# iqbal-lab-org/gramtools

Measured on AMD Instinct MI355X. Metric: 150bp reads quasimapped/sec (whole node); bit-exact coverage, higher is better.
Workload: dtype u32

## Files before the change

### gramtools_amd/csrc/gmx_engine_cover_kernels.h

```cpp
#pragma once
struct CoverAcc {
  uint32_t *acc;
  uint32_t *log;
  uint32_t *log_cursor;
  uint32_t log_cap;
  uint32_t *scratch_big;
  uint32_t n_lanes_big;
  int rng_mode;
  uint32_t log_sites;
  uint32_t *heap;
  uint64_t heap_words;
  const uint32_t *status;
  uint32_t n_tasks;
  unsigned long long *stats;
};

#define GMX_LOG_PAD 0xFFFFFFFFu
#ifdef GMX_LOOP_STATS
__device__ unsigned long long gmx_cover_stats[6 * 16];
__device__ unsigned long long gmx_coop_stats[6 * 8];
extern "C" int gmx_debug_coop_stats(unsigned long long *out, int reset) {
  if (hipMemcpyFromSymbol(out, HIP_SYMBOL(gmx_coop_stats), sizeof(gmx_coop_stats)) != hipSuccess) return -1;
  if (reset) {
    unsigned long long z[6 * 8] = {0};
// ... 808 lines not shown
    gmx_cover_single_rec<NESTED>(ix, o, acc, recs_in[i], o.cover_overflow_list, 4u);
}

__global__ void gmx_stats_limbs_kernel(unsigned long long *stats, uint32_t *limbs, int recombine) {
  const uint32_t t = threadIdx.x;
  if (!recombine) {
    if (t < 20) limbs[t] = (uint32_t)((stats[t >> 2] >> (16 * (t & 3))) & 0xFFFFull);
    else if (t < 32) limbs[t] = 0;
  } else if (t < 5) {
    unsigned long long v = 0;
    for (int l = 3; l >= 0; --l) v = (v << 16) + limbs[4 * t + l];
    stats[t] = v;
  }
}

#define GMX_PACK_READS 128
#define GMX_PACK_IN_BYTES (24 * 1024)
#define GMX_PACK_OUT_PAIRS (GMX_PACK_IN_BYTES / 32 + GMX_PACK_READS + 8)
typedef uint32_t __attribute__((aligned(1))) gmx_u32_unaligned;
__device__ __forceinline__ void pack4(uint32_t x, uint32_t &lo, uint32_t &hi, uint32_t &bad) {
  uint32_t y = x - 0x01010101u;
  bad |= ((y & ~x & 0x80808080u) | (y & 0xFCFCFCFCu));
  lo = (((y & 0x01010101u) * 0x01020408u) >> 24) & 0xFu;
  hi = ((((y >> 1) & 0x01010101u) * 0x01020408u) >> 24) & 0xFu;
}
__device__ __forceinline__ uint2 pack_tail(const uint8_t *p, uint32_t rem, uint32_t &bad) {
  uint2 out = make_uint2(0, 0);
  for (uint32_t j = 0; j < rem; ++j) {
    uint32_t x = p[j];
    if (x < 1 || x > 4) bad = 1;
    out.x |= ((x - 1u) & 1u) << j;
    out.y |= (((x - 1u) >> 1) & 1u) << j;
  }
  return out;
}
#define GMX_PACK_THREADS (2 * GMX_PACK_READS)
__global__ void __launch_bounds__(GMX_PACK_THREADS) gmx_pack_kernel(BatchView b, uint8_t *skip, uint2 *packed, uint32_t *counters,
                                                                    uint32_t *zero, uint32_t zero_words) {
  __shared__ uint4 in4[GMX_PACK_IN_BYTES / 16 + 2];
  __shared__ uint2 outp[GMX_PACK_OUT_PAIRS];
  if (blockIdx.x == 0)
    for (uint32_t i = threadIdx.x; i < GMX_N_COUNTERS * GMX_CNT_STRIDE; i += GMX_PACK_THREADS) counters[i] = 0;
  for (uint32_t i = blockIdx.x * GMX_PACK_THREADS + threadIdx.x; i < zero_words; i += gridDim.x * GMX_PACK_THREADS) zero[i] = 0;
  const uint32_t r0 = blockIdx.x * GMX_PACK_READS;
  const uint32_t r1 = min(r0 + GMX_PACK_READS, b.n_reads);
  const uint32_t read = r0 + (threadIdx.x >> 1), half = threadIdx.x & 1u;
  const uint64_t s0 = b.offsets[r0], s1 = b.offsets[r1];
  const uintptr_t g0 = reinterpret_cast<uintptr_t>(b.reads + s0);
  const uint32_t shift = (uint32_t)(g0 & 15u);
  const uint64_t span = (s1 - s0) + shift;
  if (span <= GMX_PACK_IN_BYTES) {
    const uint4 *src = reinterpret_cast<const uint4 *>(g0 - shift);
    const uint32_t n16 = (uint32_t)((span + 15) >> 4);
    {
      uint32_t i = threadIdx.x;
      for (; i + 2 * GMX_PACK_THREADS < n16; i += 3 * GMX_PACK_THREADS) {
        const uint4 v0 = src[i], v1 = src[i + GMX_PACK_THREADS], v2 = src[i + 2 * GMX_PACK_THREADS];
        in4[i] = v0;
// ... 66 lines not shown
```

### gramtools_amd/csrc/gmx_engine_debug.h

```cpp

struct GmxDebugPools {
  GmxFinalState *states = nullptr;
  uint32_t *stack = nullptr;
  GmxPathNode *arena = nullptr;
  uint32_t *result = nullptr;
  uint32_t *in = nullptr;
  uint2 *planes = nullptr;
  uint32_t cap_states = 0, cap_nodes = 0, cap_in = 0, cap_pairs = 0;
};

__global__ void __launch_bounds__(64) gmx_debug_search_kernel(GmxIndexView ix, BatchView b, const uint32_t *in, uint32_t from, uint32_t stop,
                                                              uint32_t mode, uint32_t from_seed_table, BigOut g, uint32_t *result) {
  const bool active = threadIdx.x == 0;
  BigCtx ctx;
  ctx.sp = 0;
  ctx.cap = g.max_states;
  ctx.stack = g.stack;
  ctx.arena = g.arena;
  ctx.arena_n = 0;
  ctx.arena_cap = g.max_path_nodes;
  ctx.status = GMX_TASK_MAPPED;
  ctx.out = g.states;
  ctx.n_out = 0;
  ctx.out_cap = g.max_states;
// ... 160 lines not shown
  }
  e->keep_states = on != 0;
  return GMX_OK;
} GMX_GUARD_INT("gmx_engine_debug_keep_states")

int gmx_debug_final_states(gmx_engine *e, uint64_t task, uint32_t *out, uint64_t cap_words, uint64_t *n_words, int *tier) try {
  if (!e || !n_words) {
    gmx_set_error("gmx_debug_final_states: null argument");
    return GMX_EINVAL;
  }
  if (!e->keep_states || task >= 2 * e->keep_reads) {
    gmx_set_error("gmx_debug_final_states: no such task in the last batch (gmx_engine_debug_keep_states first)");
    return GMX_EINVAL;
  }
  HIP_TRY(hipSetDevice(e->opts.device));
  HIP_TRY(hipDeviceSynchronize());
  int rc = debug_isa(e);
  if (rc) return rc;
  uint32_t raw[GMX_N_COUNTERS * GMX_CNT_STRIDE];
  HIP_TRY(hipMemcpy(raw, e->d_counters, sizeof(raw), hipMemcpyDeviceToHost));
  auto c = [&](int i) { return raw[i * GMX_CNT_STRIDE]; };
  DebugWriter w{out, cap_words};
  {
    const uint32_t n_huge = c(11);
    std::vector<uint32_t> huge(n_huge);
    if (n_huge) HIP_TRY(hipMemcpy(huge.data(), e->d_huge, n_huge * sizeof(uint32_t), hipMemcpyDeviceToHost));
    for (uint32_t t : huge)
      if (t == task) {
        gmx_set_error("gmx_debug_final_states: the task was searched by the last tier, which keeps no states");
        return GMX_ECAP;
// ... 247 lines not shown
```

### gramtools_amd/csrc/gmx_engine_host.h

```cpp
#pragma once
#define HIP_TRY(expr)                                                                      \
  do {                                                                                     \
    hipError_t _e = (expr);                                                                \
    if (_e != hipSuccess) {                                                                \
      gmx_set_error(std::string(#expr) + ": " + hipGetErrorString(_e));                    \
      return GMX_EHIP;                                                                     \
    }                                                                                      \
  } while (0)

enum : int { GMX_TK_SEED = 0, GMX_TK_FILTER0, GMX_TK_FILTER1, GMX_TK_SINGLE, GMX_TK_EXTEND2, GMX_TK_UNPACK, GMX_TK_N };
static_assert(GMX_TK_N <= GMX_TIMED_KERNELS, "gmx_timing::kernel_ms holds GMX_TIMED_KERNELS entries");

struct gmx_engine {
  gmx_engine_opts opts;
  GmxIndexView dview;
  std::vector<void *> allocs;
  uint64_t index_bytes = 0;
  uint32_t *d_fused = nullptr, *d_limbs = nullptr;
  size_t n_fused = 0, n_acc = 0;
  std::vector<uint32_t> phys_allele, phys_pb, phys_grouped;
  std::vector<uint32_t> hit_fix;
  unsigned long long *d_stats = nullptr;
  uint32_t *d_error = nullptr;
  uint32_t *d_log = nullptr, *d_log_cursor = nullptr;
// ... 33 lines not shown
  std::map<std::vector<uint32_t>, uint64_t> log_counts;
  uint32_t *h_log_state = nullptr;
  hipEvent_t ev_log_state = nullptr;
  bool log_state_pending = false;
  uint32_t *d_log_retry[2] = {nullptr, nullptr}, *d_log_retry_recs[2] = {nullptr, nullptr}, *d_log_retry_huge[2] = {nullptr, nullptr};
  int log_retry_side = 0;
  BatchView last_b{};
  SearchOut last_o{};
  CoverAcc last_acc{};
  size_t last_big_lds = 0;
  uint64_t log_replays = 0, log_replayed_entries = 0;
  uint64_t log_known = 0;
  uint64_t log_reads_since = 0;
  bool reset_pending = false;
  hipStream_t reset_stream = nullptr;
  hipStream_t side2_stream = nullptr;
  hipEvent_t ev_fork2 = nullptr, ev_side1 = nullptr, ev_filter = nullptr;
  hipStream_t side_stream = nullptr;
  hipEvent_t ev_fork = nullptr, ev_join = nullptr;
  hipEvent_t ev_wait = nullptr;
  struct GmxDeviceIndex *shared_index = nullptr;
  uint32_t filter_lds_words = 0;
  const uint32_t *d_kmer_planar = nullptr;
  const uint32_t *d_absent = nullptr;
  uint32_t n_absent = 0;
  bool use_absent = false;
  uint32_t n_cus = 256;
  uint32_t probe_iters = GMX_PROBE_ITERS;
  uint32_t extend_cap = 0;
  uint32_t extend_budget = 8;
// ... 85 lines not shown
    return GMX_OK;
  }
  int upload(const uint32_t **dst, const gmx::WordBuf &src) {
    uint32_t *q = nullptr;
    int rc = alloc(&q, src.size(), false);
    if (rc) return rc;
    const size_t piece = (size_t)1 << 28;
    for (size_t at = 0; at < src.size(); at += piece)
      HIP_TRY(hipMemcpy(q + at, src.data() + at, std::min(piece, src.size() - at) * sizeof(uint32_t), hipMemcpyHostToDevice));
    index_bytes += src.size() * sizeof(uint32_t);
    *dst = q;
    return GMX_OK;
  }
};

static hipError_t gmx_event_wait(hipEvent_t ev) {
  static const bool spin = getenv("GMX_WAIT_SPIN") != nullptr;
  if (spin) return hipEventSynchronize(ev);
  const auto t0 = std::chrono::steady_clock::now();
  for (bool napping = false;;) {
    const hipError_t q = hipEventQuery(ev);
    if (q != hipErrorNotReady) return q;
    (void)hipGetLastError();
    if (!napping) {
      napping = std::chrono::steady_clock::now() - t0 > std::chrono::microseconds(60);
      continue;
    }
    struct timespec ts = {0, 50 * 1000};
    nanosleep(&ts, nullptr);
  }
}

static int gmx_quiesce(gmx_engine *e) {
  if (!e->ev_wait) HIP_TRY(hipEventCreateWithFlags(&e->ev_wait, hipEventDisableTiming | hipEventBlockingSync));
  hipStream_t streams[5] = {e->last_stream, e->copy_stream, e->side_stream, e->side2_stream, e->copy_stream2};
  for (int i = 0; i < 5; ++i) {
    if (i > 0 && !streams[i]) continue;
    bool seen = false;
    for (int j = 0; j < i; ++j) seen = seen || streams[j] == streams[i];
    if (seen) continue;
// ... 9 lines not shown
  HIP_TRY(hipEventRecord(e->ev_zeroed, stream));
  ++e->zero_epoch;
  return GMX_OK;
}
static int twin_join(gmx_engine *e, hipStream_t stream) {
  gmx_engine *tw = e->twin;
  if (!tw || !e->twin_in_flight) return GMX_OK;
  if (!e->ev_twin_done) HIP_TRY(hipEventCreateWithFlags(&e->ev_twin_done, hipEventDisableTiming));
  HIP_TRY(hipEventRecord(e->ev_twin_done, tw->main_stream));
  HIP_TRY(hipStreamWaitEvent(stream, e->ev_twin_done, 0));
  return GMX_OK;
}
static int flush_reset(gmx_engine *e) {
  if (!e->reset_pending) return GMX_OK;
  e->reset_pending = false;
  HIP_TRY(hipMemsetAsync(e->d_fused, 0, (e->n_fused + 32) * 4, e->reset_stream));
  return note_zeroed(e, e->reset_stream);
}

static int log_settle(gmx_engine *e);
static int gmx_log_drain(gmx_engine *e, uint64_t keep_below) {
  int frc = flush_reset(e);
  if (frc) return frc;
  HIP_TRY(hipDeviceSynchronize());
  uint32_t used = 0;
  HIP_TRY(hipMemcpy(&used, e->d_log_cursor, 4, hipMemcpyDeviceToHost));
  used = std::min(used, e->log_cap);
  e->log_reads_since = 0;
  e->log_known = used;
  if (used <= keep_below) return GMX_OK;
  std::vector<uint32_t> w(used);
  HIP_TRY(hipMemcpy(w.data(), e->d_log, (size_t)used * 4, hipMemcpyDeviceToHost));
  std::vector<uint32_t> key;
// ... 448 lines not shown
  (void)hipSetDevice(e->opts.device);
  (void)hipDeviceSynchronize();
  if (e->twin) gmx_engine_destroy(e->twin);
  e->twin = nullptr;
  if (e->main_stream) (void)hipStreamDestroy(e->main_stream);
  if (e->ev_zeroed) (void)hipEventDestroy(e->ev_zeroed);
  if (e->ev_twin_done) (void)hipEventDestroy(e->ev_twin_done);
  if (e->side_stream) (void)hipStreamDestroy(e->side_stream);
  if (e->side2_stream) (void)hipStreamDestroy(e->side2_stream);
  if (e->ev_fork2) (void)hipEventDestroy(e->ev_fork2);
  if (e->ev_side1) (void)hipEventDestroy(e->ev_side1);
  if (e->ev_filter) (void)hipEventDestroy(e->ev_filter);
  if (e->ev_fork) (void)hipEventDestroy(e->ev_fork);
  if (e->ev_join) (void)hipEventDestroy(e->ev_join);
  if (e->ev_wait) (void)hipEventDestroy(e->ev_wait);
  if (e->copy_stream) (void)hipStreamDestroy(e->copy_stream);
  if (e->copy_stream2) (void)hipStreamDestroy(e->copy_stream2);
  if (e->h_log_state) (void)hipHostFree(e->h_log_state);
  if (e->ev_log_state) (void)hipEventDestroy(e->ev_log_state);
  for (auto &sl : e->pslot) {
    if (sl.copied) (void)hipEventDestroy(sl.copied);
    if (sl.done) (void)hipEventDestroy(sl.done);
  }
  for (auto &sl : e->stage) {
    if (sl.copied) (void)hipEventDestroy(sl.copied);
    if (sl.done) (void)hipEventDestroy(sl.done);
    if (sl.h_offsets) (void)hipHostFree(sl.h_offsets);
    if (sl.h_seeds) (void)hipHostFree(sl.h_seeds);
  }
  for (void *p : e->allocs) (void)hipFree(p);
  if (e->d_outcomes) (void)hipFree(e->d_outcomes);
  gmx_dev_index_release(e->shared_index);
  delete e;
} GMX_GUARD_VOID("gmx_engine_destroy")

int gmx_engine_reset(gmx_engine *e) try {
  HIP_TRY(hipSetDevice(e->opts.device));
  e->reset_pending = false;
  HIP_TRY(hipDeviceSynchronize());
  HIP_TRY(hipMemset(e->d_fused, 0, (e->n_fused + 32) * 4));
  HIP_TRY(hipMemset(e->d_error, 0, 8));
  HIP_TRY(hipMemset(e->d_counters, 0, GMX_N_COUNTERS * GMX_CNT_STRIDE * 4));
  if (e->twin) {
    HIP_TRY(hipMemset(e->twin->d_error, 0, 8));
    HIP_TRY(hipMemset(e->twin->d_counters, 0, GMX_N_COUNTERS * GMX_CNT_STRIDE * 4));
    e->twin_in_flight = false;
  }
  if (e->outcome_count) HIP_TRY(hipMemset(e->d_outcomes, 0, (e->outcome_count + 3) & ~3ull));
  e->outcome_count = 0;
  ++e->outcome_epoch;
  e->log_counts.clear();
  e->log_known = e->log_reads_since = 0;
  e->log_state_pending = false;
  return GMX_OK;
} GMX_GUARD_INT("gmx_engine_reset")

int gmx_engine_reset_async(gmx_engine *e, void *hip_stream) try {
  HIP_TRY(hipSetDevice(e->opts.device));
  hipStream_t st = (hipStream_t)hip_stream;
  int frc = flush_reset(e);
  if (frc) return frc;
  if ((frc = twin_join(e, st))) return frc;
  e->twin_in_flight = false;
  if (e->outcome_count) HIP_TRY(hipMemsetAsync(e->d_outcomes, 0, (e->outcome_count + 3) & ~3ull, st));
  e->outcome_count = 0;
  ++e->outcome_epoch;
  e->reset_pending = true;
  e->reset_stream = st;
  e->log_counts.clear();
  e->log_known = e->log_reads_since = 0;
  e->log_state_pending = false;
  return GMX_OK;
} GMX_GUARD_INT("gmx_engine_reset_async")

static bool gmx_ab_no_filter() {
  static const bool off = getenv("GMX_AB_NO_FILTER") != nullptr;
// ... 77 lines not shown
  }
}

struct BatchInput {
  const uint8_t *d_reads = nullptr;
  const uint64_t *d_offsets = nullptr;
  const uint32_t *d_seeds = nullptr;
  const uint2 *d_planes = nullptr;
  const uint8_t *d_skip = nullptr;
  const uint32_t *d_twobit = nullptr;
  uint32_t twobit_base0 = 0;
  uint32_t uniform_len = 0;
  uint64_t n_reads = 0, total_bases = 0;
};

__global__ void gmx_batch_begin_kernel(uint32_t *counters, uint32_t *zero, uint32_t zero_words) {
  if (blockIdx.x == 0)
    for (uint32_t i = threadIdx.x; i < GMX_N_COUNTERS * GMX_CNT_STRIDE; i += blockDim.x) counters[i] = 0;
  for (uint32_t i = blockIdx.x * blockDim.x + threadIdx.x; i < zero_words; i += gridDim.x * blockDim.x) zero[i] = 0;
}

__device__ __forceinline__ uint32_t gmx_even_bits(unsigned long long x) {
  x &= 0x5555555555555555ull;
  x = (x | (x >> 1)) & 0x3333333333333333ull;
  x = (x | (x >> 2)) & 0x0F0F0F0F0F0F0F0Full;
  x = (x | (x >> 4)) & 0x00FF00FF00FF00FFull;
  x = (x | (x >> 8)) & 0x0000FFFF0000FFFFull;
  x = (x | (x >> 16)) & 0x00000000FFFFFFFFull;
  return (uint32_t)x;
}
__global__ void __launch_bounds__(256) gmx_unpack2_kernel(BatchView b, const uint32_t *stream, uint32_t base0, uint2 *packed) {
  const uint32_t ppr_uniform = b.pairs_per_read;
  for (uint64_t t = blockIdx.x * (uint64_t)blockDim.x + threadIdx.x;; t += (uint64_t)gridDim.x * blockDim.x) {
// ... 27 lines not shown
  }
}

static int launch_batch(gmx_engine *e, const BatchInput &in, hipStream_t stream) {
  const uint64_t n_reads = in.n_reads, total_bases = in.total_bases;
  if (n_reads == 0) return GMX_OK;
  if (n_reads > (0x7fffffffull / GMX_FAST_ARENA) / 2) {
    gmx_set_error("batch too large: at most 44 M reads per launch (lower gmx_engine_opts.max_batch_reads)");
    return GMX_EINVAL;
  }
  int rc = e->log_sites ? log_settle(e) : GMX_OK;
  if (rc) return rc;
  if ((rc = ensure_batch_capacity(e, n_reads, true))) return rc;
  const bool fold_reset = e->reset_pending && e->reset_stream == stream;
  if (e->reset_pending && !fold_reset && (rc = flush_reset(e))) return rc;
  e->reset_pending = false;
  if (!in.d_planes) {
    uint64_t need = total_bases / 32 + n_reads + 16;
    if (need > e->cap_packed) {
      rc = e->alloc(&e->d_packed, need, false);
      if (rc) return rc;
      e->cap_packed = need;
    }
  }
  BatchView b{in.d_reads, in.d_offsets, in.d_seeds, (in.d_planes || in.d_twobit) ? in.d_skip : e->d_skip, in.d_planes ? in.d_planes : e->d_packed,
              (uint32_t)n_reads, (uint32_t)(e->opts.forward_only ? 1 : 0), in.uniform_len, (in.uniform_len + 31u) / 32u,
              e->keep_states ? 1u : 0u};
  const uint32_t region_inv = (uint32_t)std::min<uint64_t>(0xFFFFFFFFull, (((uint64_t)GMX_REGIONS << 32) + e->dview.n_prg - 1) / std::max<uint32_t>(e->dview.n_prg, 1u));
  SearchOut o{};
  o.status = e->d_status;
  o.n_final = e->d_n_final;
// ... 68 lines not shown
    HIP_TRY(hipEventCreate(&ev.c));
    for (int k = 0; k < GMX_TK_N; ++k) {
      HIP_TRY(hipEventCreate(&ev.k[k][0]));
      HIP_TRY(hipEventCreate(&ev.k[k][1]));
    }
    ev.reads = n_reads;
    HIP_TRY(hipEventRecord(ev.s, stream));
  }
  auto t_ev = [&](int k, int side) -> hipEvent_t {
    if (!e->timing) return nullptr;
    ev.timed |= 1u << k;
    return ev.k[k][side];
  };
  if (in.d_planes || in.d_twobit) {
    hipLaunchKernelGGL(gmx_batch_begin_kernel, dim3(fold_reset ? 256 : 1), dim3(1024), 0, stream, e->d_counters,
                       fold_reset ? e->d_fused : nullptr, fold_reset ? (uint32_t)(e->n_fused + 32) : 0u);
    if (in.d_twobit) {
      const uint64_t threads = in.uniform_len ? n_reads * ((in.uniform_len + 31u) / 32u) : n_reads;
      hipExtLaunchKernelGGL(gmx_unpack2_kernel, dim3((unsigned)std::min<uint64_t>((threads + 255) / 256, 1u << 20)), dim3(256), 0, stream,
                            t_ev(GMX_TK_UNPACK, 0), t_ev(GMX_TK_UNPACK, 1), 0u, b, in.d_twobit, in.twobit_base0, e->d_packed);
    }
  } else
    hipLaunchKernelGGL(gmx_pack_kernel, dim3((unsigned)((n_reads + GMX_PACK_READS - 1) / GMX_PACK_READS)), dim3(GMX_PACK_THREADS), 0, stream, b,
                       e->d_skip, e->d_packed, e->d_counters, fold_reset ? e->d_fused : nullptr, fold_reset ? (uint32_t)(e->n_fused + 32) : 0u);
  if (fold_reset && (rc = note_zeroed(e, stream))) return rc;
  size_t lds = (size_t)GMX_STACK_DEPTH * GMX_STACK_WORDS * GMX_BLOCK * sizeof(uint32_t);
  const size_t big_lds = (size_t)GMX_BIG_LDS_DEPTH * GMX_STACK_WORDS * 64 * sizeof(uint32_t);
  dim3 task_grid((n_tasks + GMX_BLOCK - 1) / GMX_BLOCK);
  const bool seeded = e->dview.kmer_size2 != 0 && !getenv("GMX_NO_SEEDED");
  if (seeded)
    hipExtLaunchKernelGGL(gmx_seed_kernel, dim3((n_tasks + GMX_SEED_THREADS * GMX_SEED_CHUNKS - 1) / (GMX_SEED_THREADS * GMX_SEED_CHUNKS)), dim3(GMX_SEED_THREADS), 0, stream,
                          t_ev(GMX_TK_SEED, 0), t_ev(GMX_TK_SEED, 1), 0u, e->dview, b, o);
  else if (e->seed_cursor)
    hipExtLaunchKernelGGL(gmx_probe_kernel<true>, task_grid, dim3(GMX_BLOCK), (uint32_t)lds, stream, t_ev(GMX_TK_SEED, 0), t_ev(GMX_TK_SEED, 1), 0u, e->dview, b, o,
                          e->probe_iters);
  else
    hipExtLaunchKernelGGL(gmx_probe_kernel<false>, task_grid, dim3(GMX_BLOCK), (uint32_t)lds, stream, t_ev(GMX_TK_SEED, 0), t_ev(GMX_TK_SEED, 1), 0u, e->dview, b, o,
                          e->probe_iters);
  HIP_TRY(hipEventRecord(e->ev_fork, stream));
// ... 297 lines not shown
  out->eng = tw;
  out->stream = tw->main_stream;
  e->twin_in_flight = true;
  e->last_on_twin = true;
  return GMX_OK;
}

static int map_reads_packed_impl(gmx_engine *e, const uint64_t *planes, bool twobit, const uint64_t *offsets, uint32_t uniform_len,
                                 const uint32_t *seeds, const uint8_t *skip, uint64_t n_reads) {
  if (!e || !planes || !seeds || (!offsets && !uniform_len)) {
    gmx_set_error("gmx_map_reads_packed_host / gmx_map_reads_2bit_host: null argument (offsets may be null only with uniform_len)");
    return GMX_EINVAL;
  }
  if (n_reads == 0) return GMX_OK;
  HIP_TRY(hipSetDevice(e->opts.device));
  if (!e->copy_stream) HIP_TRY(hipStreamCreateWithFlags(&e->copy_stream, hipStreamNonBlocking));
  static const bool two_copy_streams = getenv("GMX_TWO_COPY_STREAMS") != nullptr;
  if (two_copy_streams && !e->copy_stream2) HIP_TRY(hipStreamCreateWithFlags(&e->copy_stream2, hipStreamNonBlocking));
  const uint32_t ppr = (uniform_len + 31u) / 32u;
  auto base_at = [&](uint64_t r) -> uint64_t { return uniform_len ? r * uniform_len : offsets[r] - offsets[0]; };
  auto pair_at = [&](uint64_t r) -> uint64_t {
    if (twobit) return (base_at(r) + 31) >> 5;
    return uniform_len ? r * ppr : ((offsets[r] >> 5) - (offsets[0] >> 5)) + r;
  };
  struct Reg { const void *p; bool on; };
  Reg regs[4] = {{planes, false}, {offsets, false}, {seeds, false}, {skip, false}};
  const uint64_t reg_bytes[4] = {pair_at(n_reads) * 8, (n_reads + 1) * 8, n_reads * 4, n_reads};
  bool all_pinned = true;
  for (int i = 0; i < 4; ++i) {
    if (!regs[i].p || gmx_is_pinned(regs[i].p)) continue;
// ... 88 lines not shown
  }
  } catch (...) {
    rc = gmx_guard_catch(twobit ? "gmx_map_reads_2bit_host" : "gmx_map_reads_packed_host");
  }
  if (rc != GMX_OK || !all_pinned) {
    (void)hipStreamSynchronize(e->copy_stream);
    if (e->copy_stream2) (void)hipStreamSynchronize(e->copy_stream2);
    if (rc != GMX_OK) {
      (void)hipDeviceSynchronize();
      for (auto &sl : e->pslot) sl.busy = false;
    }
  }
  for (int i = 0; i < 4; ++i)
    if (regs[i].on) (void)hipHostUnregister(const_cast<void *>(regs[i].p));
  (void)hipGetLastError();
  return rc;
}

int gmx_map_reads_packed_host(gmx_engine *e, const uint64_t *planes, const uint64_t *offsets, uint32_t uniform_len,
                              const uint32_t *seeds, const uint8_t *skip, uint64_t n_reads) try {
  return map_reads_packed_impl(e, planes, false, offsets, uniform_len, seeds, skip, n_reads);
} GMX_GUARD_INT("gmx_map_reads_packed_host")

static uint64_t gmx_feed_chunk(const gmx_engine *e) {
  static const char *env = getenv("GMX_FEED_CHUNK");
  if (env) return std::max<uint64_t>(1, std::min<uint64_t>(e->opts.max_batch_reads, strtoull(env, nullptr, 10)));
  return e->opts.max_batch_reads;
}

int gmx_map_reads_packed_device(gmx_engine *e, const uint64_t *d_planes, const uint64_t *d_offsets, uint32_t uniform_len,
// ... 49 lines not shown
int gmx_engine_seeds_in_place(gmx_engine *e, int on) try {
  if (!e) {
    gmx_set_error("null engine");
    return GMX_EINVAL;
  }
  e->seeds_in_place = on != 0;
  return GMX_OK;
} GMX_GUARD_INT("gmx_engine_seeds_in_place")

int gmx_engine_sync_uploads(gmx_engine *e) try {
  if (!e) {
    gmx_set_error("null engine");
    return GMX_EINVAL;
  }
  HIP_TRY(hipSetDevice(e->opts.device));
  if (e->copy_stream) {
    if (!e->ev_wait) HIP_TRY(hipEventCreateWithFlags(&e->ev_wait, hipEventDisableTiming | hipEventBlockingSync));
    HIP_TRY(hipEventRecord(e->ev_wait, e->copy_stream));
    HIP_TRY(gmx_event_wait(e->ev_wait));
  }
  if (e->copy_stream2) {
    if (!e->ev_wait) HIP_TRY(hipEventCreateWithFlags(&e->ev_wait, hipEventDisableTiming | hipEventBlockingSync));
    HIP_TRY(hipEventRecord(e->ev_wait, e->copy_stream2));
    HIP_TRY(gmx_event_wait(e->ev_wait));
  }
  return GMX_OK;
} GMX_GUARD_INT("gmx_engine_sync_uploads")

static std::mutex g_host_mu;
struct HostBlock {
// ... 107 lines not shown
      sl.d_offsets = nullptr;
      sl.d_seeds = nullptr;
      sl.d_skip = nullptr;
      sl.cap_reads = 0;
      if ((rc = e->alloc(&sl.d_offsets, n_reads + 1, false)) || (rc = e->alloc(&sl.d_seeds, n_reads, false)) ||
          (rc = e->alloc(&sl.d_skip, n_reads, false)))
        return rc;
      sl.cap_reads = n_reads;
    }
  }
  return GMX_OK;
} GMX_GUARD_INT("gmx_engine_reserve_packed")

int gmx_engine_sync(gmx_engine *e) try {
  HIP_TRY(hipSetDevice(e->opts.device));
  {
    int frc = flush_reset(e);
    if (frc) return frc;
    if ((frc = log_settle(e))) return frc;
  }
  {
    int qrc = gmx_quiesce(e);
    if (qrc) return qrc;
    if (e->twin && (qrc = gmx_quiesce(e->twin))) return qrc;
    e->twin_in_flight = false;
  }
  HIP_TRY(hipStreamSynchronize(e->last_stream));
  HIP_TRY(hipDeviceSynchronize());
  uint32_t c[4] = {0, 0, 0, 0};
  HIP_TRY(hipMemcpy(c + 2, e->d_error, 8, hipMemcpyDeviceToHost));
  if (c[2] == 0 && e->twin) {
    HIP_TRY(hipMemcpy(c + 2, e->twin->d_error, 8, hipMemcpyDeviceToHost));
    if (c[2] != 0) HIP_TRY(hipMemset(e->twin->d_error, 0, 8));
  }
  if (c[2] != 0) {
    HIP_TRY(hipMemset(e->d_error, 0, 8));
    char msg[256];
    if (c[2] == GMX_TASK_LOGFULL) {
      snprintf(msg, sizeof(msg),
               "a read's records exceed the whole grouped-allele-count log (sites without dense group counters; %u words): "
               "nothing of it was recorded: raise gmx_engine_opts.log_cap_words",
               e->log_cap);
      gmx_set_error(msg);
      return GMX_ECAP;
    }
    if (c[2] == GMX_TASK_OVERFLOW) {
      snprintf(msg, sizeof(msg),
               "read %u (orientation %u) needs more memory for its search states or its mapping instances than the whole "
               "last-tier heap holds (%llu bytes); nothing of this read was recorded: raise gmx_engine_opts.huge_heap_bytes "
               "(GMX_HUGE_HEAP_BYTES)",
// ... 57 lines not shown
  out->cover_launches = e->cover_launches;
  out->reads = e->timed_reads;
  for (int k = 0; k < GMX_TIMED_KERNELS; ++k) {
    out->kernel_ms[k] = e->kernel_ms[k];
    out->kernel_launches[k] = e->kernel_launches[k];
    e->kernel_ms[k] = 0;
    e->kernel_launches[k] = 0;
  }
  e->search_ms = e->cover_ms = 0;
  e->search_launches = e->cover_launches = e->timed_reads = 0;
  return GMX_OK;
} GMX_GUARD_INT("gmx_engine_timing")

int gmx_engine_queue_counts(gmx_engine *e, gmx_queue_counts *out) try {
  HIP_TRY(hipSetDevice(e->opts.device));
  HIP_TRY(hipDeviceSynchronize());
  uint32_t raw[GMX_N_COUNTERS * GMX_CNT_STRIDE];
  HIP_TRY(hipMemcpy(raw, (e->twin && e->last_on_twin ? e->twin : e)->d_counters, sizeof(raw), hipMemcpyDeviceToHost));
  auto c = [&](int i) { return (uint64_t)raw[i * GMX_CNT_STRIDE]; };
  out->mapped = 0;
  for (int r = 0; r < GMX_REGIONS; ++r) out->mapped += c(16 + r);
  out->mapped += c(8);
  out->alive = c(5);
  out->dead = c(6) + c(12);
  out->overflow_probe = c(1);
  out->overflow_extend = c(9);
  out->big_mapped = c(7);
  out->cover_general = c(8);
  out->cover_mid = c(13);
  out->cover_overflow = c(4);
// ... 5 lines not shown
  out->log_replayed_entries = e->log_replayed_entries;
  out->overflow_split = c(29);
  return GMX_OK;
} GMX_GUARD_INT("gmx_engine_queue_counts")

int gmx_coverage_device(gmx_engine *e, gmx_device_coverage *out) try {
  {
    int frc = flush_reset(e);
    if (frc) return frc;
  }
  if (e->twin && e->twin_in_flight) {
    int qrc = gmx_quiesce(e->twin);
    if (qrc) return qrc;
    e->twin_in_flight = false;
  }
  out->allele_sum = out->per_base = out->grouped = nullptr;
  out->n_allele_sum = e->n_allele;
  out->n_per_base = e->n_pb;
  out->n_grouped = e->n_grouped;
  out->stats = e->d_stats;
  out->n_stats = 5;
  out->fused = e->d_fused;
  out->n_fused = e->n_fused;
  return GMX_OK;
} GMX_GUARD_INT("gmx_coverage_device")

int gmx_coverage_reduce_begin(gmx_engine *e, void *hip_stream) try {
  if (!e) {
    gmx_set_error("null engine");
    return GMX_EINVAL;
  }
  {
    int frc = flush_reset(e);
    if (frc) return frc;
    if ((frc = log_settle(e))) return frc;
  }
  HIP_TRY(hipSetDevice(e->opts.device));
  {
    int trc = twin_join(e, (hipStream_t)hip_stream);
    if (trc) return trc;
  }
  hipLaunchKernelGGL(gmx_stats_limbs_kernel, dim3(1), dim3(64), 0, (hipStream_t)hip_stream, e->d_stats, e->d_limbs, 0);
  HIP_TRY(hipGetLastError());
  return GMX_OK;
} GMX_GUARD_INT("gmx_coverage_reduce_begin")

int gmx_coverage_reduce_end(gmx_engine *e, void *hip_stream) try {
  if (!e) {
    gmx_set_error("null engine");
    return GMX_EINVAL;
  }
  {
    int frc = flush_reset(e);
    if (frc) return frc;
  }
  HIP_TRY(hipSetDevice(e->opts.device));
  hipLaunchKernelGGL(gmx_stats_limbs_kernel, dim3(1), dim3(64), 0, (hipStream_t)hip_stream, e->d_stats, e->d_limbs, 1);
  HIP_TRY(hipGetLastError());
  return GMX_OK;
} GMX_GUARD_INT("gmx_coverage_reduce_end")

int gmx_coverage_fetch(gmx_engine *e, uint32_t *allele_sum, uint32_t *per_base, uint32_t *grouped, gmx_stats *stats) try {
  if (!e) {
    gmx_set_error("null engine");
    return GMX_EINVAL;
  }
  {
    int frc = flush_reset(e);
    if (frc) return frc;
    if ((frc = log_settle(e))) return frc;
  }
  HIP_TRY(hipSetDevice(e->opts.device));
  HIP_TRY(hipDeviceSynchronize());
  std::vector<uint32_t> block(std::max<size_t>(e->n_acc, 1));
  if (e->n_acc) HIP_TRY(hipMemcpy(block.data(), e->d_fused, e->n_acc * 4, hipMemcpyDeviceToHost));
  if (allele_sum) for (size_t i = 0; i < e->phys_allele.size(); ++i) allele_sum[i] = block[e->phys_allele[i]];
  if (per_base) for (size_t i = 0; i < e->phys_pb.size(); ++i) per_base[i] = block[e->phys_pb[i]];
  if (grouped) for (size_t i = 0; i < e->phys_grouped.size(); ++i) grouped[i] = block[e->phys_grouped[i]];
  for (size_t i = 0; i + 3 < e->hit_fix.size(); i += 4) {
    const uint32_t hits = block[e->hit_fix[i]];
    if (allele_sum) allele_sum[e->hit_fix[i + 1]] += hits;
    if (grouped) grouped[e->hit_fix[i + 2]] += hits;
    if (per_base) per_base[e->hit_fix[i + 3]] += hits;
  }
  if (stats) {
    unsigned long long s[5];
    HIP_TRY(hipMemcpy(s, e->d_stats, sizeof(s), hipMemcpyDeviceToHost));
    stats->all_reads_count = s[0];
    stats->skipped_reads_count = s[1];
    stats->missing_kmer_reads_count = s[2];
    stats->no_extension_reads_count = s[3];
    stats->exact_mapped_reads_count = s[4];
  }
  return GMX_OK;
} GMX_GUARD_INT("gmx_coverage_fetch")

int gmx_engine_record_outcomes(gmx_engine *e, int on) try {
  if (!e) {
    gmx_set_error("null engine");
    return GMX_EINVAL;
  }
  e->record_outcomes = on != 0;
  return GMX_OK;
} GMX_GUARD_INT("gmx_engine_record_outcomes")

int64_t gmx_engine_outcome_count(gmx_engine *e) try {
  if (!e) {
    gmx_set_error("null engine");
// ... 13 lines not shown
    return GMX_EINVAL;
  }
  {
    int frc = flush_reset(e);
    if (frc) return frc;
    if ((frc = log_settle(e))) return frc;
  }
  HIP_TRY(hipSetDevice(e->opts.device));
  HIP_TRY(hipDeviceSynchronize());
  if (n) HIP_TRY(hipMemcpy(out, reinterpret_cast<const uint8_t *>(e->d_outcomes) + first, n, hipMemcpyDeviceToHost));
  return GMX_OK;
} GMX_GUARD_INT("gmx_engine_fetch_outcomes")

int64_t gmx_coverage_fetch_grouped_log(gmx_engine *e, uint32_t *out, uint64_t cap_words) try {
  if (!e) return GMX_EINVAL;
  if (hipSetDevice(e->opts.device) != hipSuccess) return GMX_EHIP;
  if (log_settle(e)) return GMX_EHIP;
  if (gmx_log_drain(e, 0)) return GMX_EHIP;
  uint64_t n = 0;
  for (auto const &kv : e->log_counts) {
    const uint64_t words = 4 + (kv.first.size() - 1);
    if (out && n + words <= cap_words) {
      out[n] = kv.first[0];
      out[n + 1] = (uint32_t)(kv.first.size() - 1) | GMX_LOG_COUNTED;
      out[n + 2] = (uint32_t)kv.second;
      out[n + 3] = (uint32_t)(kv.second >> 32);
      for (size_t j = 1; j < kv.first.size(); ++j) out[n + 3 + j] = kv.first[j];
    }
    n += words;
  }
  return (int64_t)n;
} GMX_GUARD_INT("gmx_coverage_fetch_grouped_log")

// ... 4 lines not shown
  }
  {
    int frc = flush_reset(e);
    if (frc) return frc;
  }
  HIP_TRY(hipSetDevice(e->opts.device));
  return gmx_engine_log_import(e, records, (size_t)n_words, replace != 0);
} GMX_GUARD_INT("gmx_coverage_import_grouped_log")

}

uint64_t gmx_engine_outcome_epoch(const gmx_engine *e) { return e->outcome_epoch; }

void gmx_engine_raw(gmx_engine *e, GmxEngineRaw *out) {
  (void)flush_reset(e);
  out->device = e->opts.device;
  out->d_fused = e->d_fused;
  out->n_fused = e->n_fused;
  out->log_sites = e->log_sites;
}

int gmx_engine_log_export(gmx_engine *e, std::vector<uint32_t> &out) {
  {
    int frc = flush_reset(e);
    if (frc) return frc;
    if ((frc = log_settle(e))) return frc;
  }
  const int64_t n = gmx_coverage_fetch_grouped_log(e, nullptr, 0);
  if (n < 0) return (int)n;
  out.assign((size_t)n, 0);
// ... 38 lines not shown
```

Measured before the change: 1.450 billion.

## Gather coverage on device, defer whole resets, and skip redundant syncs

```diff
diff --git a/gramtools_amd/csrc/gmx_engine_cover_kernels.h b/gramtools_amd/csrc/gmx_engine_cover_kernels.h
--- a/gramtools_amd/csrc/gmx_engine_cover_kernels.h
+++ b/gramtools_amd/csrc/gmx_engine_cover_kernels.h
@@ -846,6 +846,33 @@
   }
 }
 
+#define GMX_GATHER_TAIL 16u
+__global__ void __launch_bounds__(256) gmx_gather_slots_kernel(const uint32_t *block, const uint32_t *phys, uint32_t n_slots, uint32_t *out,
+                                                               const uint32_t *stats_words, const uint32_t *err, const uint32_t *err_twin,
+                                                               const uint32_t *log_cursor) {
+  for (uint32_t i = blockIdx.x * blockDim.x + threadIdx.x; i < n_slots; i += gridDim.x * blockDim.x) out[i] = block[phys[i]];
+  if (blockIdx.x == 0 && threadIdx.x < GMX_GATHER_TAIL) {
+    const uint32_t t = threadIdx.x;
+    uint32_t v = 0;
+    if (t < 10) v = stats_words[t];
+    else if (t < 12) v = err[t - 10];
+    else if (t < 14) v = err_twin ? err_twin[t - 12] : 0u;
+    else if (t == 14) v = *log_cursor;
+    out[n_slots + t] = v;
+  }
+}
+__global__ void __launch_bounds__(256) gmx_gather_hits_kernel(const uint32_t *block, const uint4 *fix, uint32_t n_fix, uint32_t *out,
+                                                              uint32_t n_allele, uint32_t n_pb) {
+  for (uint32_t i = blockIdx.x * blockDim.x + threadIdx.x; i < n_fix; i += gridDim.x * blockDim.x) {
+    const uint4 f = fix[i];
+    const uint32_t hits = block[f.x];
+    if (hits == 0) continue;
+    atomicAdd(out + f.y, hits);
+    atomicAdd(out + n_allele + n_pb + f.z, hits);
+    atomicAdd(out + n_allele + f.w, hits);
+  }
+}
+
 #define GMX_PACK_READS 128
 #define GMX_PACK_IN_BYTES (24 * 1024)
 #define GMX_PACK_OUT_PAIRS (GMX_PACK_IN_BYTES / 32 + GMX_PACK_READS + 8)
@@ -868,12 +895,13 @@
 }
 #define GMX_PACK_THREADS (2 * GMX_PACK_READS)
 __global__ void __launch_bounds__(GMX_PACK_THREADS) gmx_pack_kernel(BatchView b, uint8_t *skip, uint2 *packed, uint32_t *counters,
-                                                                    uint32_t *zero, uint32_t zero_words) {
+                                                                    uint32_t *zero, uint32_t zero_words, uint32_t *zero_err) {
   __shared__ uint4 in4[GMX_PACK_IN_BYTES / 16 + 2];
   __shared__ uint2 outp[GMX_PACK_OUT_PAIRS];
   if (blockIdx.x == 0)
     for (uint32_t i = threadIdx.x; i < GMX_N_COUNTERS * GMX_CNT_STRIDE; i += GMX_PACK_THREADS) counters[i] = 0;
   for (uint32_t i = blockIdx.x * GMX_PACK_THREADS + threadIdx.x; i < zero_words; i += gridDim.x * GMX_PACK_THREADS) zero[i] = 0;
+  if (zero_err && blockIdx.x == 0 && threadIdx.x < 2) zero_err[threadIdx.x] = 0;
   const uint32_t r0 = blockIdx.x * GMX_PACK_READS;
   const uint32_t r1 = min(r0 + GMX_PACK_READS, b.n_reads);
   const uint32_t read = r0 + (threadIdx.x >> 1), half = threadIdx.x & 1u;
diff --git a/gramtools_amd/csrc/gmx_engine_debug.h b/gramtools_amd/csrc/gmx_engine_debug.h
--- a/gramtools_amd/csrc/gmx_engine_debug.h
+++ b/gramtools_amd/csrc/gmx_engine_debug.h
@@ -198,6 +198,10 @@
     return GMX_EINVAL;
   }
   HIP_TRY(hipSetDevice(e->opts.device));
+  {
+    int frc = flush_reset(e);
+    if (frc) return frc;
+  }
   HIP_TRY(hipDeviceSynchronize());
   int rc = debug_isa(e);
   if (rc) return rc;
diff --git a/gramtools_amd/csrc/gmx_engine_host.h b/gramtools_amd/csrc/gmx_engine_host.h
--- a/gramtools_amd/csrc/gmx_engine_host.h
+++ b/gramtools_amd/csrc/gmx_engine_host.h
@@ -71,6 +71,15 @@
   uint64_t log_reads_since = 0;
   bool reset_pending = false;
   hipStream_t reset_stream = nullptr;
+  bool reset_whole = false;
+  hipEvent_t ev_order = nullptr;
+  hipStream_t ext_stream = nullptr;
+  bool busy = true, exported = false;
+  uint32_t seen_error[4] = {0, 0, 0, 0};
+  int gather_state = 0;
+  uint32_t *d_gather_phys = nullptr, *d_gather_fix = nullptr, *d_result = nullptr, *h_result = nullptr;
+  size_t n_result = 0;
+  hipEvent_t ev_fetch = nullptr;
   hipStream_t side2_stream = nullptr;
   hipEvent_t ev_fork2 = nullptr, ev_side1 = nullptr, ev_filter = nullptr;
   hipStream_t side_stream = nullptr;
@@ -186,7 +195,7 @@
   }
 };
 
-static hipError_t gmx_event_wait(hipEvent_t ev) {
+static hipError_t gmx_event_wait(hipEvent_t ev, uint32_t spin_us = 60) {
   static const bool spin = getenv("GMX_WAIT_SPIN") != nullptr;
   if (spin) return hipEventSynchronize(ev);
   const auto t0 = std::chrono::steady_clock::now();
@@ -195,7 +204,7 @@
     if (q != hipErrorNotReady) return q;
     (void)hipGetLastError();
     if (!napping) {
-      napping = std::chrono::steady_clock::now() - t0 > std::chrono::microseconds(60);
+      napping = std::chrono::steady_clock::now() - t0 > std::chrono::microseconds(spin_us);
       continue;
     }
     struct timespec ts = {0, 50 * 1000};
@@ -235,9 +244,47 @@
 static int flush_reset(gmx_engine *e) {
   if (!e->reset_pending) return GMX_OK;
   e->reset_pending = false;
+  e->busy = true;
+  if (e->reset_whole) {
+    e->reset_whole = false;
+    HIP_TRY(hipDeviceSynchronize());
+    HIP_TRY(hipMemsetAsync(e->d_fused, 0, (e->n_fused + 32) * 4, nullptr));
+    HIP_TRY(hipMemsetAsync(e->d_error, 0, 8, nullptr));
+    HIP_TRY(hipMemsetAsync(e->d_counters, 0, GMX_N_COUNTERS * GMX_CNT_STRIDE * 4, nullptr));
+    HIP_TRY(hipStreamSynchronize(nullptr));
+    return GMX_OK;
+  }
   HIP_TRY(hipMemsetAsync(e->d_fused, 0, (e->n_fused + 32) * 4, e->reset_stream));
   return note_zeroed(e, e->reset_stream);
 }
+static int null_stream_behind(gmx_engine *e, hipStream_t st) {
+  if (!st) return GMX_OK;
+  if (!e->ev_order) HIP_TRY(hipEventCreateWithFlags(&e->ev_order, hipEventDisableTiming));
+  HIP_TRY(hipEventRecord(e->ev_order, st));
+  HIP_TRY(hipStreamWaitEvent(nullptr, e->ev_order, 0));
+  return GMX_OK;
+}
+
+struct GmxJobTrace {
+  bool on = getenv("GMX_JOB_TRACE") != nullptr;
+  std::vector<std::pair<const char *, std::chrono::steady_clock::time_point>> marks;
+  void mark(const char *what) {
+    if (on) marks.emplace_back(what, std::chrono::steady_clock::now());
+  }
+  void dump() {
+    if (!on || marks.empty()) return;
+    std::string line = "GMX_JOB_TRACE";
+    for (size_t i = 0; i < marks.size(); ++i) {
+      char buf[96];
+      snprintf(buf, sizeof(buf), " %s=%.1f", marks[i].first,
+               std::chrono::duration<double, std::micro>(marks[i].second - marks[0].second).count());
+      line += buf;
+    }
+    fprintf(stderr, "%s\n", line.c_str());
+    marks.clear();
+  }
+};
+static GmxJobTrace g_job_trace;
 
 static int log_settle(gmx_engine *e);
 static int gmx_log_drain(gmx_engine *e, uint64_t keep_below) {
@@ -716,6 +763,9 @@
   if (e->ev_fork) (void)hipEventDestroy(e->ev_fork);
   if (e->ev_join) (void)hipEventDestroy(e->ev_join);
   if (e->ev_wait) (void)hipEventDestroy(e->ev_wait);
+  if (e->ev_order) (void)hipEventDestroy(e->ev_order);
+  if (e->ev_fetch) (void)hipEventDestroy(e->ev_fetch);
+  if (e->h_result) (void)hipHostFree(e->h_result);
   if (e->copy_stream) (void)hipStreamDestroy(e->copy_stream);
   if (e->copy_stream2) (void)hipStreamDestroy(e->copy_stream2);
   if (e->h_log_state) (void)hipHostFree(e->h_log_state);
@@ -738,7 +788,30 @@
 
 int gmx_engine_reset(gmx_engine *e) try {
   HIP_TRY(hipSetDevice(e->opts.device));
+  g_job_trace.mark("reset");
+  e->busy = true;
+  static const bool eager = getenv("GMX_EAGER_RESET") != nullptr;
+  if (!e->twin && !eager) {
+    int rc = GMX_OK;
+    if (e->reset_pending && !e->reset_whole) {
+      const hipStream_t st = e->reset_stream;
+      if ((rc = flush_reset(e)) || (rc = null_stream_behind(e, st))) return rc;
+    }
+    if ((rc = null_stream_behind(e, e->last_stream)) || (rc = null_stream_behind(e, e->ext_stream))) return rc;
+    if (e->outcome_count) HIP_TRY(hipMemsetAsync(e->d_outcomes, 0, (e->outcome_count + 3) & ~3ull, nullptr));
+    e->outcome_count = 0;
+    ++e->outcome_epoch;
+    e->reset_pending = true;
+    e->reset_whole = true;
+    e->reset_stream = nullptr;
+    e->log_counts.clear();
+    e->log_known = e->log_reads_since = 0;
+    e->log_state_pending = false;
+    g_job_trace.mark("reset_end");
+    return GMX_OK;
+  }
   e->reset_pending = false;
+  e->reset_whole = false;
   HIP_TRY(hipDeviceSynchronize());
   HIP_TRY(hipMemset(e->d_fused, 0, (e->n_fused + 32) * 4));
   HIP_TRY(hipMemset(e->d_error, 0, 8));
@@ -754,6 +827,7 @@
   e->log_counts.clear();
   e->log_known = e->log_reads_since = 0;
   e->log_state_pending = false;
+  g_job_trace.mark("reset_end");
   return GMX_OK;
 } GMX_GUARD_INT("gmx_engine_reset")
 
@@ -762,6 +836,7 @@
   hipStream_t st = (hipStream_t)hip_stream;
   int frc = flush_reset(e);
   if (frc) return frc;
+  e->busy = true;
   if ((frc = twin_join(e, st))) return frc;
   e->twin_in_flight = false;
   if (e->outcome_count) HIP_TRY(hipMemsetAsync(e->d_outcomes, 0, (e->outcome_count + 3) & ~3ull, st));
@@ -869,9 +944,10 @@
   uint64_t n_reads = 0, total_bases = 0;
 };
 
-__global__ void gmx_batch_begin_kernel(uint32_t *counters, uint32_t *zero, uint32_t zero_words) {
+__global__ void gmx_batch_begin_kernel(uint32_t *counters, uint32_t *zero, uint32_t zero_words, uint32_t *zero_err) {
   if (blockIdx.x == 0)
     for (uint32_t i = threadIdx.x; i < GMX_N_COUNTERS * GMX_CNT_STRIDE; i += blockDim.x) counters[i] = 0;
+  if (zero_err && blockIdx.x == 0 && threadIdx.x < 2) zero_err[threadIdx.x] = 0;
   for (uint32_t i = blockIdx.x * blockDim.x + threadIdx.x; i < zero_words; i += gridDim.x * blockDim.x) zero[i] = 0;
 }
 
@@ -929,7 +1005,10 @@
   if ((rc = ensure_batch_capacity(e, n_reads, true))) return rc;
   const bool fold_reset = e->reset_pending && e->reset_stream == stream;
   if (e->reset_pending && !fold_reset && (rc = flush_reset(e))) return rc;
+  uint32_t *const fold_err = fold_reset && e->reset_whole ? e->d_error : nullptr;
   e->reset_pending = false;
+  e->reset_whole = false;
+  (e->owner ? e->owner : e)->busy = true;
   if (!in.d_planes) {
     uint64_t need = total_bases / 32 + n_reads + 16;
     if (need > e->cap_packed) {
@@ -1028,7 +1107,7 @@
   };
   if (in.d_planes || in.d_twobit) {
     hipLaunchKernelGGL(gmx_batch_begin_kernel, dim3(fold_reset ? 256 : 1), dim3(1024), 0, stream, e->d_counters,
-                       fold_reset ? e->d_fused : nullptr, fold_reset ? (uint32_t)(e->n_fused + 32) : 0u);
+                       fold_reset ? e->d_fused : nullptr, fold_reset ? (uint32_t)(e->n_fused + 32) : 0u, fold_err);
     if (in.d_twobit) {
       const uint64_t threads = in.uniform_len ? n_reads * ((in.uniform_len + 31u) / 32u) : n_reads;
       hipExtLaunchKernelGGL(gmx_unpack2_kernel, dim3((unsigned)std::min<uint64_t>((threads + 255) / 256, 1u << 20)), dim3(256), 0, stream,
@@ -1036,7 +1115,7 @@
     }
   } else
     hipLaunchKernelGGL(gmx_pack_kernel, dim3((unsigned)((n_reads + GMX_PACK_READS - 1) / GMX_PACK_READS)), dim3(GMX_PACK_THREADS), 0, stream, b,
-                       e->d_skip, e->d_packed, e->d_counters, fold_reset ? e->d_fused : nullptr, fold_reset ? (uint32_t)(e->n_fused + 32) : 0u);
+                       e->d_skip, e->d_packed, e->d_counters, fold_reset ? e->d_fused : nullptr, fold_reset ? (uint32_t)(e->n_fused + 32) : 0u, fold_err);
   if (fold_reset && (rc = note_zeroed(e, stream))) return rc;
   size_t lds = (size_t)GMX_STACK_DEPTH * GMX_STACK_WORDS * GMX_BLOCK * sizeof(uint32_t);
   const size_t big_lds = (size_t)GMX_BIG_LDS_DEPTH * GMX_STACK_WORDS * 64 * sizeof(uint32_t);
@@ -1364,6 +1443,8 @@
   }
   if (n_reads == 0) return GMX_OK;
   HIP_TRY(hipSetDevice(e->opts.device));
+  g_job_trace.mark("feed");
+  e->busy = true;
   if (!e->copy_stream) HIP_TRY(hipStreamCreateWithFlags(&e->copy_stream, hipStreamNonBlocking));
   static const bool two_copy_streams = getenv("GMX_TWO_COPY_STREAMS") != nullptr;
   if (two_copy_streams && !e->copy_stream2) HIP_TRY(hipStreamCreateWithFlags(&e->copy_stream2, hipStreamNonBlocking));
@@ -1482,6 +1563,7 @@
   for (int i = 0; i < 4; ++i)
     if (regs[i].on) (void)hipHostUnregister(const_cast<void *>(regs[i].p));
   (void)hipGetLastError();
+  g_job_trace.mark("feed_end");
   return rc;
 }
 
@@ -1561,6 +1643,7 @@
     return GMX_EINVAL;
   }
   HIP_TRY(hipSetDevice(e->opts.device));
+  if (!e->busy) return GMX_OK;
   if (e->copy_stream) {
     if (!e->ev_wait) HIP_TRY(hipEventCreateWithFlags(&e->ev_wait, hipEventDisableTiming | hipEventBlockingSync));
     HIP_TRY(hipEventRecord(e->ev_wait, e->copy_stream));
@@ -1698,6 +1781,12 @@
 
 int gmx_engine_sync(gmx_engine *e) try {
   HIP_TRY(hipSetDevice(e->opts.device));
+  g_job_trace.mark("sync");
+  if (!e->busy && !e->exported && !e->reset_pending && !e->log_state_pending && !(e->seen_error[0] | e->seen_error[2])) {
+    g_job_trace.mark("sync_end");
+    g_job_trace.dump();
+    return GMX_OK;
+  }
   {
     int frc = flush_reset(e);
     if (frc) return frc;
@@ -1709,15 +1798,23 @@
     if (e->twin && (qrc = gmx_quiesce(e->twin))) return qrc;
     e->twin_in_flight = false;
   }
+  g_job_trace.mark("sync_quiesced");
   HIP_TRY(hipStreamSynchronize(e->last_stream));
   HIP_TRY(hipDeviceSynchronize());
+  e->busy = false;
+  e->ext_stream = nullptr;
+  memset(e->seen_error, 0, sizeof(e->seen_error));
+  g_job_trace.mark("sync_device_idle");
   uint32_t c[4] = {0, 0, 0, 0};
   HIP_TRY(hipMemcpy(c + 2, e->d_error, 8, hipMemcpyDeviceToHost));
+  g_job_trace.mark("sync_end");
+  g_job_trace.dump();
   if (c[2] == 0 && e->twin) {
     HIP_TRY(hipMemcpy(c + 2, e->twin->d_error, 8, hipMemcpyDeviceToHost));
     if (c[2] != 0) HIP_TRY(hipMemset(e->twin->d_error, 0, 8));
   }
   if (c[2] != 0) {
+    e->busy = e->twin != nullptr;
     HIP_TRY(hipMemset(e->d_error, 0, 8));
     char msg[256];
     if (c[2] == GMX_TASK_LOGFULL) {
@@ -1805,6 +1902,10 @@
 
 int gmx_engine_queue_counts(gmx_engine *e, gmx_queue_counts *out) try {
   HIP_TRY(hipSetDevice(e->opts.device));
+  {
+    int frc = flush_reset(e);
+    if (frc) return frc;
+  }
   HIP_TRY(hipDeviceSynchronize());
   uint32_t raw[GMX_N_COUNTERS * GMX_CNT_STRIDE];
   HIP_TRY(hipMemcpy(raw, (e->twin && e->last_on_twin ? e->twin : e)->d_counters, sizeof(raw), hipMemcpyDeviceToHost));
@@ -1840,6 +1941,7 @@
     if (qrc) return qrc;
     e->twin_in_flight = false;
   }
+  e->exported = true;
   out->allele_sum = out->per_base = out->grouped = nullptr;
   out->n_allele_sum = e->n_allele;
   out->n_per_base = e->n_pb;
@@ -1866,6 +1968,8 @@
     int trc = twin_join(e, (hipStream_t)hip_stream);
     if (trc) return trc;
   }
+  e->busy = true;
+  e->ext_stream = (hipStream_t)hip_stream;
   hipLaunchKernelGGL(gmx_stats_limbs_kernel, dim3(1), dim3(64), 0, (hipStream_t)hip_stream, e->d_stats, e->d_limbs, 0);
   HIP_TRY(hipGetLastError());
   return GMX_OK;
@@ -1881,25 +1985,109 @@
     if (frc) return frc;
   }
   HIP_TRY(hipSetDevice(e->opts.device));
+  e->busy = true;
+  e->ext_stream = (hipStream_t)hip_stream;
   hipLaunchKernelGGL(gmx_stats_limbs_kernel, dim3(1), dim3(64), 0, (hipStream_t)hip_stream, e->d_stats, e->d_limbs, 1);
   HIP_TRY(hipGetLastError());
   return GMX_OK;
 } GMX_GUARD_INT("gmx_coverage_reduce_end")
+
+#define GMX_GATHER_BUDGET (256ull << 20)
+static void gather_setup(gmx_engine *e) {
+  e->gather_state = -1;
+  if (getenv("GMX_HOST_GATHER")) return;
+  const uint64_t n_slots = (uint64_t)e->phys_allele.size() + e->phys_pb.size() + e->phys_grouped.size();
+  const uint64_t n_fix = e->hit_fix.size() / 4;
+  if (e->phys_allele.size() != e->n_allele || e->phys_pb.size() != e->n_pb || e->phys_grouped.size() != e->n_grouped) return;
+  if (n_slots * 8 + n_fix * 16 + GMX_GATHER_TAIL * 4 > GMX_GATHER_BUDGET) return;
+  for (const std::vector<uint32_t> *t : {&e->phys_allele, &e->phys_pb, &e->phys_grouped})
+    for (uint32_t v : *t)
+      if (v >= e->n_acc) return;
+  for (uint64_t i = 0; i < n_fix; ++i)
+    if (e->hit_fix[4 * i] >= e->n_acc || e->hit_fix[4 * i + 1] >= e->n_allele || e->hit_fix[4 * i + 2] >= e->n_grouped ||
+        e->hit_fix[4 * i + 3] >= e->n_pb)
+      return;
+  std::vector<uint32_t> phys;
+  phys.reserve(n_slots);
+  phys.insert(phys.end(), e->phys_allele.begin(), e->phys_allele.end());
+  phys.insert(phys.end(), e->phys_pb.begin(), e->phys_pb.end());
+  phys.insert(phys.end(), e->phys_grouped.begin(), e->phys_grouped.end());
+  const size_t n_result = (size_t)n_slots + GMX_GATHER_TAIL;
+  bool ok = e->alloc(&e->d_gather_phys, (size_t)n_slots, false) == GMX_OK && e->alloc(&e->d_gather_fix, (size_t)n_fix * 4, false) == GMX_OK &&
+            e->alloc(&e->d_result, n_result, true) == GMX_OK &&
+            hipHostMalloc(reinterpret_cast<void **>(&e->h_result), n_result * 4, hipHostMallocDefault) == hipSuccess &&
+            hipEventCreateWithFlags(&e->ev_fetch, hipEventDisableTiming) == hipSuccess;
+  if (ok && n_slots) ok = hipMemcpy(e->d_gather_phys, phys.data(), n_slots * 4, hipMemcpyHostToDevice) == hipSuccess;
+  if (ok && n_fix) ok = hipMemcpy(e->d_gather_fix, e->hit_fix.data(), n_fix * 16, hipMemcpyHostToDevice) == hipSuccess;
+  if (!ok) {
+    (void)hipGetLastError();
+    return;
+  }
+  e->n_result = n_result;
+  e->gather_state = 1;
+}
+
+static int coverage_fetch_device(gmx_engine *e, uint32_t *allele_sum, uint32_t *per_base, uint32_t *grouped, gmx_stats *stats) {
+  int rc;
+  if ((rc = null_stream_behind(e, e->last_stream)) || (rc = null_stream_behind(e, e->ext_stream))) return rc;
+  if ((rc = twin_join(e, nullptr))) return rc;
+  const uint32_t n_slots = (uint32_t)(e->n_result - GMX_GATHER_TAIL), n_fix = (uint32_t)(e->hit_fix.size() / 4);
+  hipLaunchKernelGGL(gmx_gather_slots_kernel, dim3(std::max(1u, std::min((n_slots + 255u) / 256u, e->n_cus * 8u))), dim3(256), 0, nullptr, e->d_fused,
+                     e->d_gather_phys, n_slots, e->d_result, reinterpret_cast<const uint32_t *>(e->d_stats), e->d_error,
+                     e->twin ? e->twin->d_error : nullptr, e->d_log_cursor);
+  if (n_fix)
+    hipLaunchKernelGGL(gmx_gather_hits_kernel, dim3(std::min((n_fix + 255u) / 256u, e->n_cus * 8u)), dim3(256), 0, nullptr, e->d_fused,
+                       reinterpret_cast<const uint4 *>(e->d_gather_fix), n_fix, e->d_result, e->n_allele, e->n_pb);
+  HIP_TRY(hipGetLastError());
+  HIP_TRY(hipMemcpyAsync(e->h_result, e->d_result, e->n_result * 4, hipMemcpyDeviceToHost, nullptr));
+  HIP_TRY(hipEventRecord(e->ev_fetch, nullptr));
+  g_job_trace.mark("fetch_enqueued");
+  HIP_TRY(gmx_event_wait(e->ev_fetch, 1000));
+  g_job_trace.mark("fetch_waited");
+  const uint32_t *r = e->h_result;
+  if (allele_sum) memcpy(allele_sum, r, (size_t)e->n_allele * 4);
+  if (per_base) memcpy(per_base, r + e->n_allele, (size_t)e->n_pb * 4);
+  if (grouped) memcpy(grouped, r + e->n_allele + e->n_pb, (size_t)e->n_grouped * 4);
+  const uint32_t *tail = r + n_slots;
+  if (stats) {
+    unsigned long long sw[5];
+    memcpy(sw, tail, sizeof(sw));
+    stats->all_reads_count = sw[0];
+    stats->skipped_reads_count = sw[1];
+    stats->missing_kmer_reads_count = sw[2];
+    stats->no_extension_reads_count = sw[3];
+    stats->exact_mapped_reads_count = sw[4];
+  }
+  memcpy(e->seen_error, tail + 10, sizeof(e->seen_error));
+  e->twin_in_flight = false;
+  e->ext_stream = nullptr;
+  e->busy = false;
+  return GMX_OK;
+}
 
 int gmx_coverage_fetch(gmx_engine *e, uint32_t *allele_sum, uint32_t *per_base, uint32_t *grouped, gmx_stats *stats) try {
   if (!e) {
     gmx_set_error("null engine");
     return GMX_EINVAL;
   }
+  g_job_trace.mark("fetch");
+  HIP_TRY(hipSetDevice(e->opts.device));
   {
     int frc = flush_reset(e);
     if (frc) return frc;
     if ((frc = log_settle(e))) return frc;
   }
-  HIP_TRY(hipSetDevice(e->opts.device));
+  if (e->gather_state == 0) gather_setup(e);
+  if (e->gather_state == 1) {
+    const int rc = coverage_fetch_device(e, allele_sum, per_base, grouped, stats);
+    g_job_trace.mark("fetch_end");
+    return rc;
+  }
   HIP_TRY(hipDeviceSynchronize());
+  g_job_trace.mark("fetch_device_idle");
   std::vector<uint32_t> block(std::max<size_t>(e->n_acc, 1));
   if (e->n_acc) HIP_TRY(hipMemcpy(block.data(), e->d_fused, e->n_acc * 4, hipMemcpyDeviceToHost));
+  g_job_trace.mark("fetch_block_copied");
   if (allele_sum) for (size_t i = 0; i < e->phys_allele.size(); ++i) allele_sum[i] = block[e->phys_allele[i]];
   if (per_base) for (size_t i = 0; i < e->phys_pb.size(); ++i) per_base[i] = block[e->phys_pb[i]];
   if (grouped) for (size_t i = 0; i < e->phys_grouped.size(); ++i) grouped[i] = block[e->phys_grouped[i]];
@@ -1909,6 +2097,7 @@
     if (grouped) grouped[e->hit_fix[i + 2]] += hits;
     if (per_base) per_base[e->hit_fix[i + 3]] += hits;
   }
+  g_job_trace.mark("fetch_gathered");
   if (stats) {
     unsigned long long s[5];
     HIP_TRY(hipMemcpy(s, e->d_stats, sizeof(s), hipMemcpyDeviceToHost));
@@ -1918,6 +2107,7 @@
     stats->no_extension_reads_count = s[3];
     stats->exact_mapped_reads_count = s[4];
   }
+  g_job_trace.mark("fetch_end");
   return GMX_OK;
 } GMX_GUARD_INT("gmx_coverage_fetch")
 
@@ -1961,9 +2151,12 @@
 
 int64_t gmx_coverage_fetch_grouped_log(gmx_engine *e, uint32_t *out, uint64_t cap_words) try {
   if (!e) return GMX_EINVAL;
-  if (hipSetDevice(e->opts.device) != hipSuccess) return GMX_EHIP;
-  if (log_settle(e)) return GMX_EHIP;
-  if (gmx_log_drain(e, 0)) return GMX_EHIP;
+  g_job_trace.mark("fetch_log");
+  if (e->log_sites) {
+    if (hipSetDevice(e->opts.device) != hipSuccess) return GMX_EHIP;
+    if (log_settle(e)) return GMX_EHIP;
+    if (gmx_log_drain(e, 0)) return GMX_EHIP;
+  }
   uint64_t n = 0;
   for (auto const &kv : e->log_counts) {
     const uint64_t words = 4 + (kv.first.size() - 1);
@@ -1998,6 +2191,7 @@
 
 void gmx_engine_raw(gmx_engine *e, GmxEngineRaw *out) {
   (void)flush_reset(e);
+  e->exported = true;
   out->device = e->opts.device;
   out->d_fused = e->d_fused;
   out->n_fused = e->n_fused;
```

Result: no change. 1.440 billion (-0.7%).
